# byteowlz/kokorox

Measured on NVIDIA B200. Metric: audio-seconds per second, higher is better.
Workload: dtype bf16

## Files before the change

### kokorox_b200/csrc/kernels.h

```cpp
#pragma once
#include "common.h"
#include <cuda_bf16.h>

namespace kkx {

enum Act : int { ACT_NONE = 0, ACT_LRELU = 1, ACT_SNAKE = 2, ACT_GELU_NEW = 3 };

struct ConvArgs {
  const float* in = nullptr; int ldi = 0;
  const int* in_off = nullptr; const int* in_len = nullptr;
  const int* m_len = nullptr; int max_m = 0; int B = 1;
  long long sum_m = 0;
  const float* w = nullptr; const float* bias = nullptr;
  int Ci = 0, Co = 0, ks = 1, dil = 1, pad = 0, stride = 1;
  const float* pscale = nullptr; const float* pshift = nullptr; int pld = 0;
  int pact = ACT_NONE; float pslope = 0.f; const float* palpha = nullptr;
  float* out = nullptr; int ldo = 0; int ocol = 0; const int* out_off = nullptr;
  int ors = 1, oro = 0;
  int eact = ACT_NONE;
  const float* res = nullptr; int ldr = 0; int rcol = 0; const int* res_off = nullptr;
  int res_shift = 0;
  float oscale = 1.f; int accumulate = 0;
};
void launch_conv_f32(const ConvArgs& a, cudaStream_t st);

struct TcConvArgs {
  const void* tmA = nullptr;
  const void* tmB = nullptr;
  const void* tmA2 = nullptr;
  const void* tmB2 = nullptr;
  const void* tmB_c = nullptr;
  const void* tmB2_c = nullptr;
  int debug = 0;
  int tf32 = 0;
  int nprod = 3;
  int f16 = 0;
  float wscale = 1.f;
  int eact = ACT_NONE;
  int Cpad = 0, Ci = 0, Co = 0, ks = 1, dil = 1, pad = 0;
  const int* in_off = nullptr; const int* m_len = nullptr; int max_m = 0; int B = 1; long long sum_m = 0;
  const float* bias = nullptr;
  float* out = nullptr; int ldo = 0; int ocol = 0; const int* out_off = nullptr; int ors = 1, oro = 0;
  const float* res = nullptr; int ldr = 0; int rcol = 0; const int* res_off = nullptr; int res_shift = 0;
  float oscale = 1.f; int accumulate = 0; int vec4 = 0;
  long long* timing = nullptr;
  const int* tile_start = nullptr; int ntiles_m = 0;
  int group_m = 1;
  void* out_hi = nullptr; void* out_lo = nullptr; int out_pl_ld = 0;
  void* attn_pl[6] = {nullptr, nullptr, nullptr, nullptr, nullptr, nullptr};
  int pair = 0;
  int force_kernel = 0;
  int nphase = 1;
  int phase_pad[10] = {0};
  int phase_oro[10] = {0};
  int phase_loop = 0;
};
void launch_conv_tc(const TcConvArgs& a, cudaStream_t st);
bool conv_tc_takes_pair(const TcConvArgs& a);
void make_tmap_bf16(void* out_map, const void* ptr, long long inner, long long outer,
                    long long pitch_elems, int box_outer);
void make_tmap_f32(void* out_map, const void* ptr, long long inner, long long outer,
                   long long pitch_elems, int box_outer);
void make_tmap_f16(void* out_map, const void* ptr, long long inner, long long outer,
                   long long pitch_elems, int box_outer);
inline int tc_box_n(int Co) { return Co > 128 ? 256 : (Co > 64 ? 128 : 64); }
inline int tc_box_n_tf32(int Co) { return Co > 64 ? 128 : 64; }
void launch_apply_tf32(const float* x, int ldx, int C, const float* scale, const float* shift, int act,
                       float slope, float* out_hi, float* out_lo, int Cpad, int rows_total,
                       const int* off, const int* len, int B, int max_len, cudaStream_t st);
constexpr float kSplitF16Scale = 16.f;
float split_f16_host(const float* w, size_t n, unsigned short* hi, unsigned short* lo);
void launch_apply_f16x2(const float* x, int ldx, int C, const float* scale, const float* shift, int act,
                        float slope, void* out_hi, void* out_lo, int Cpad, int rows_total,
                        const int* off, const int* len, int B, int max_len, cudaStream_t st);
void launch_apply_bf16(const float* x, int ldx, int C, const float* scale, const float* shift, int act,
                       float slope, const float* alpha, void* out, int Cpad, int rows_total,
                       const int* off, const int* len, int B, int max_len, cudaStream_t st);
void launch_im2col_bf16(const float* in, int ldi, int C, int ks, int stride, int pad, void* out, int Cpad,
                        int rows_total, const int* in_off, const int* in_len, const int* out_off,
                        const int* out_len, int B, int max_out_len, cudaStream_t st, int force_generic = 0);
void launch_pool_up_bf16(const float* in, int ldi, const float* scale, const float* shift, float slope,
                         const float* w, const float* bias, int C, void* out, int Cpad, int rows_total,
                         const int* in_off, const int* in_len, const int* out_off, int B, int max_len,
                         cudaStream_t st);

struct ArbConvArgs {
  const void* x = nullptr; int in_bf16 = 0;
  const float* scale = nullptr; const float* shift = nullptr;
  const float* alpha = nullptr;
  const void* tmB = nullptr;
  int C = 0, ks = 1, dil = 1, pad = 0;
  const int* off = nullptr; const int* len = nullptr;
  const int* tile_start = nullptr;
  int B = 1; int total_tiles = 0; long long sum_m = 0;
  const float* bias = nullptr;
  __nv_bfloat16* out_bf16 = nullptr;
  float* out_f32 = nullptr;
  const float* res = nullptr; float oscale = 1.f; int accumulate = 0;
  int res_bf16 = 0;
  float* part = nullptr; int nchunk = 0;
  long long* timing = nullptr;
  int debug = 0;
  int post = 0, cout = 0, ldo = 0; float slope = 0.f;
};
int arb_tile_rows(int C);
bool arb_conv_supported(int C, int ks, int dil, int B);
void launch_arb_conv(const ArbConvArgs& a, cudaStream_t st);

struct LnArgs {
  const float* x = nullptr; int ldx = 0;
  const float* res = nullptr; int ldr = 0;
  const float* w = nullptr; const float* b = nullptr;
  const float* ada = nullptr; int ada_ld = 0; int ada_off = 0;
  float eps = 1e-5f; float slope = 1.f;
  float* out = nullptr; int ldo = 0; int ocol = 0;
  const int* off = nullptr; const int* len = nullptr; int B = 1; int max_len = 0; int C = 0;
  void* pl_hi = nullptr; void* pl_lo = nullptr; int pl_ld = 0;
};
void launch_layernorm(const LnArgs& a, cudaStream_t st);

void launch_albert_embed(const int* ids, const float* word, const float* pos, const float* type,
                         const float* lnw, const float* lnb, float* out, const int* off,
                         const int* len, int B, int max_len, cudaStream_t st);
void launch_embed_rows(const int* ids, const float* table, int C, float* out, int ldo,
                       const int* off, const int* len, int B, int max_len, cudaStream_t st);
void launch_bcast_cols(const float* vec, int ldv, int voff, int C, float* out, int ldo, int ocol,
                       const int* off, const int* len, int B, int max_len, cudaStream_t st);
void launch_copy_cols(const float* src, int lds, int scol, float* dst, int ldd, int dcol, int C,
                      const int* off, const int* len, int B, int max_len, cudaStream_t st);
void launch_add_rows(const float* a, const float* b, float* out, int C, const int* off,
                     const int* len, int B, int max_len, cudaStream_t st);
void launch_copy_row(float* u, int C, int dst_row, int src_row, const int* off, int B,
                     cudaStream_t st);

void launch_attention(const float* qkv, float* ctx, const int* off, const int* len, int B,
                      int max_len, cudaStream_t st);

size_t attention_umma_scratch_floats(int rows_total, int B);
void attention_timing_dump();
void launch_attention_umma(const float* qkv, float* scratch, float* ctx, const int* off, const int* len, int B,
                           int max_len, int rows_total, cudaStream_t st, bool planes_ready = false);
void attention_umma_planes(float* scratch, int rows_total, int B, void* (&pl)[6]);

void launch_lstm(const float* xproj, const float* whhT, float* out, int ldo, int ocol,
                 const int* off, const int* len, int B, cudaStream_t st, int variant = 1);

constexpr int kStatRows = 128;
// ... 75 lines not shown
```

### kokorox_b200/csrc/kernels_arb.cu

```cuda
#include "kernels.h"
#include "tc_ptx.cuh"
#include <type_traits>
#include <cstdlib>

namespace kkx {

namespace {

#ifdef KKX_ARB_TIMING
#define TIM_DECL(n) long long tim_acc[n] = {0}; long long tim_last = clock64(); const bool tim_on = a.timing && blockIdx.x == 0
#define TICK(slot) do { if (tim_on) { const long long now_ = clock64(); tim_acc[slot] += now_ - tim_last; tim_last = now_; } } while (0)
#define TIM_FLUSH(base, n) do { if (tim_on) for (int i_ = 0; i_ < (n); i_++) atomicAdd(reinterpret_cast<unsigned long long*>(a.timing) + (base) + i_, (unsigned long long)tim_acc[i_]); } while (0)
#else
#define TIM_DECL(n)
#define TICK(slot)
#define TIM_FLUSH(base, n)
#endif

#ifdef KKX_EXPERIMENTS
#define ARB_DBG(a, bit) ((a).debug & (bit))
#else
#define ARB_DBG(a, bit) (0)
#endif

constexpr int kArbThreads = 512;
constexpr int kArbMaxB = 512;

template <int BN>
struct ArbCfg {
  static constexpr bool T = BN == 128;
  static constexpr int MSUB = T ? 2 : 1;
  static constexpr int KCH = BN / 64;
  static constexpr int RA = MSUB * 128 + 56;
  static constexpr uint32_t A_SLOT = RA * 128;
  static constexpr int NA = 3;
  static constexpr uint32_t B_STAGE = BN * 128;
  static constexpr int NB = T ? 6 : 3;
  static constexpr int PITCH = 36;
  static constexpr uint32_t STG = T ? 0 : 2 * 128 * PITCH * 4;
  static constexpr uint32_t STAT = 4 * BN * 2 * 4;
  static constexpr uint32_t COEF = 3 * BN * 4;
  static constexpr int NBAR = 2 * NA + 2 * NB + 4;
  static constexpr uint32_t SMEM = NA * A_SLOT + NB * B_STAGE + STG + STAT + COEF + NBAR * 8 + 16 + (3 * kArbMaxB + 2) * 4 + 1024;
  static_assert(A_SLOT % 1024 == 0, "A slot must keep the 1024-byte swizzle alignment");
};

__device__ __forceinline__ uint32_t pack_bf16(float lo, float hi) {
  __nv_bfloat162 p = __floats2bfloat162_rn(lo, hi);
  return *reinterpret_cast<uint32_t*>(&p);
}

struct TileCur {
  int b, mt;
  __device__ __forceinline__ void init(const int* ts, int B, int tile) {
    int lo = 0, hi = B;
    while (hi - lo > 1) {
      const int mid = (lo + hi) >> 1;
      if (ts[mid] <= tile) lo = mid; else hi = mid;
    }
    b = lo; mt = tile - ts[lo];
  }
  __device__ __forceinline__ void next(const int* ts) {
    mt++;
    while (ts[b] + mt >= ts[b + 1]) { b++; mt = 0; if (ts[b] < 0) break; }
  }
};

template <int BN, bool CONV2, bool POST = false, int SB = 0, bool PB = false>
__global__ void __launch_bounds__(kArbThreads, 1) arb_conv_kernel(const __grid_constant__ CUtensorMap tmB, ArbConvArgs a) {
  using Cfg = ArbCfg<BN>;
  constexpr bool T = Cfg::T;
  constexpr int MSUB = Cfg::MSUB;
  static_assert(SB == 0 || (!POST && (CONV2 || SB == 1)), "stream-bf16 variants: conv1 SB=1, conv2 SB=1 (bf16 out) / SB=2 (fp32 out)");
  static_assert(!PB || (T && !CONV2 && !POST && SB == 0), "balanced-producer variant: conv1, transposed accumulator, fp32 input");
  constexpr bool XIN_BF = CONV2 || SB != 0;
  constexpr bool OUT_BF = !CONV2 || SB == 1;
  static_assert(!POST || (T && !CONV2), "post variant: transposed accumulator, fp32 input");
  constexpr int NEW = PB ? 4 : 8;
  constexpr int NPW = PB ? 8 : 14 - NEW;
  constexpr int kProdThreads = NPW * 32;
  constexpr int kProdRows = kProdThreads / 8;
  constexpr int KCH = Cfg::KCH, NA = Cfg::NA, NB = Cfg::NB, PITCH = Cfg::PITCH;
  constexpr int MT = MSUB * 128;
  extern __shared__ uint8_t smem_raw[];
  const uint32_t base = (smem_u32(smem_raw) + 1023u) & ~1023u;
  uint8_t* const gbase = smem_raw + (base - smem_u32(smem_raw));
  const uint32_t a_base = base;
  const uint32_t b_base = a_base + NA * Cfg::A_SLOT;
  const uint32_t stg_base = b_base + NB * Cfg::B_STAGE;
  const uint32_t stat_base = stg_base + Cfg::STG;
  const uint32_t coef_base = stat_base + Cfg::STAT;
  const uint32_t bar_base = coef_base + Cfg::COEF;
  const uint32_t tmem_slot = bar_base + Cfg::NBAR * 8;
  const uint32_t ts_base = tmem_slot + 16;
  auto fullA = [&](int s) { return bar_base + s * 8; };
  auto emptyA = [&](int s) { return bar_base + (NA + s) * 8; };
  auto fullB = [&](int s) { return bar_base + (2 * NA + s) * 8; };
  auto emptyB = [&](int s) { return bar_base + (2 * NA + NB + s) * 8; };
  auto tfull = [&](int j) { return bar_base + (2 * NA + 2 * NB + j) * 8; };
  auto tempty = [&](int j) { return bar_base + (2 * NA + 2 * NB + 2 + j) * 8; };
  int* const s_ts = reinterpret_cast<int*>(gbase + (ts_base - base));
  int* const s_len = s_ts + (kArbMaxB + 2);
  int* const s_off = s_len + kArbMaxB;

  const int warp = threadIdx.x >> 5, lane = threadIdx.x & 31;
  const int B = a.B;
#pragma unroll 1
  for (int i = threadIdx.x; i <= B + 1; i += kArbThreads) s_ts[i] = i <= B ? a.tile_start[i] : -1;
#pragma unroll 1
  for (int i = threadIdx.x; i < B; i += kArbThreads) { s_len[i] = a.len[i]; s_off[i] = a.off[i]; }

  if (warp == 0 && lane == 0) {
    asm volatile("prefetch.tensormap [%0];" ::"l"(&tmB) : "memory");
    for (int s = 0; s < NA; s++) { mbar_init(fullA(s), kProdThreads / 32); mbar_init(emptyA(s), 1); }
    for (int s = 0; s < NB; s++) { mbar_init(fullB(s), 1); mbar_init(emptyB(s), 1); }
    for (int j = 0; j < 2; j++) { mbar_init(tfull(j), 1); mbar_init(tempty(j), NEW); }
    asm volatile("fence.mbarrier_init.release.cluster;" ::: "memory");
    asm volatile("fence.proxy.async.shared::cta;" ::: "memory");
  }
  if (warp == 1) {
    asm volatile("tcgen05.alloc.cta_group::1.sync.aligned.shared::cta.b32 [%0], %1;" ::"r"(tmem_slot), "r"(512u) : "memory");
    asm volatile("tcgen05.relinquish_alloc_permit.cta_group::1.sync.aligned;" ::: "memory");
  }
  tc_fence_before();
  __syncthreads();
  tc_fence_after();
  uint32_t tmem_base;
  asm volatile("ld.shared.b32 %0, [%1];" : "=r"(tmem_base) : "r"(tmem_slot) : "memory");

  const int t_begin = (int)(((long long)a.total_tiles * blockIdx.x) / gridDim.x);
  const int t_end = (int)(((long long)a.total_tiles * (blockIdx.x + 1)) / gridDim.x);
  const int ks = a.ks, dil = a.dil, pad = a.pad;

  if (warp == 0) {
    if (lane == 0 && t_begin < t_end) {
      int g = 0;
      TIM_DECL(2);
      const bool resident = KCH * ks <= NB;
#pragma unroll 1
      for (int tile = t_begin; tile < (resident ? t_begin + 1 : t_end); tile++) {
#pragma unroll 1
        for (int c = 0; c < KCH; c++)
#pragma unroll 1
          for (int tap = 0; tap < ks; tap++, g++) {
            const int s = g % NB;
            mbar_wait(emptyB(s), (((uint32_t)(g / NB)) & 1u) ^ 1u);
            TICK(0);
            mbar_expect_tx(fullB(s), Cfg::B_STAGE);
            tma_load_2d(b_base + s * Cfg::B_STAGE, &tmB, tap * BN + c * 64, 0, fullB(s));
            TICK(1);
          }
      }
      TIM_FLUSH(0, 2);
    }
  } else if (warp == 1) {
    if (lane == 0 && t_begin < t_end) {
      constexpr uint32_t idesc = umma_idesc_bf16(128, BN);
      int gA = 0, gB = 0, ti = 0;
      TileCur cur;
      cur.init(s_ts, B, t_begin);
      const bool resident = KCH * ks <= NB;
      TIM_DECL(4);
#pragma unroll 1
      for (int tile = t_begin; tile < t_end; tile++, ti++) {
        const int rem = s_len[cur.b] - cur.mt * MT;
        (void)rem;
        const int buf = ti & 1;
        mbar_wait(tempty(buf), (((uint32_t)(ti >> 1)) & 1u) ^ 1u);
        tc_fence_after();
        TICK(0);
#pragma unroll 1
        for (int c = 0; c < KCH; c++, gA++) {
          const int sa = gA % NA;
          mbar_wait(fullA(sa), ((uint32_t)(gA / NA)) & 1u);
          tc_fence_after();
          TICK(1);
          const uint32_t slot = a_base + sa * Cfg::A_SLOT;
#pragma unroll 1
          for (int tap = 0; tap < ks; tap++, gB++) {
            const int sb = resident ? c * ks + tap : gB % NB;
            if (!resident || ti == 0) {
              mbar_wait(fullB(sb), resident ? 0u : ((uint32_t)(gB / NB)) & 1u);
              tc_fence_after();
            }
            TICK(2);
            const uint64_t bd = umma_desc_sw128(b_base + sb * Cfg::B_STAGE);
            if (T) {
              constexpr uint32_t idescT = umma_idesc_bf16(128, 256);
              const uint64_t xd = umma_desc_sw128(slot + (uint32_t)(tap * dil) * 128u);
              const uint32_t td = tmem_base + (uint32_t)(buf * 256);
#pragma unroll
              for (int k = 0; k < 4; k++)
                if (!ARB_DBG(a, 8)) umma_bf16(td, bd + (uint64_t)(2 * k), xd + (uint64_t)(2 * k), idescT, (c | tap | k) ? 1u : 0u);
            } else {
#pragma unroll
              for (int sub = 0; sub < MSUB; sub++) {
                if (sub * 128 >= rem) continue;
                const uint64_t ad = umma_desc_sw128(slot + (uint32_t)(sub * 128 + tap * dil) * 128u);
                const uint32_t td = tmem_base + (uint32_t)((buf * MSUB + sub) * BN);
#pragma unroll
                for (int k = 0; k < 4; k++)
                  umma_bf16(td, ad + (uint64_t)(2 * k), bd + (uint64_t)(2 * k), idesc, (c | tap | k) ? 1u : 0u);
              }
            }
            if (!resident) umma_commit(emptyB(sb));
            TICK(3);
          }
          umma_commit(emptyA(sa));
        }
        umma_commit(tfull(buf));
        cur.next(s_ts);
      }
      TIM_FLUSH(4, 4);
    }
  } else if (T && warp < 2 + NEW) {
    const int eg = (warp - 2) >> 2;
    const int q = warp & 3;
    const int co = q * 32 + lane;
    const float bias_c = a.bias[co];
    const float2 bias2 = make_float2(bias_c, bias_c);
    const float2 os2 = make_float2(a.oscale, a.oscale);
    const bool accum = a.accumulate != 0;
    constexpr int RW = MSUB * 128 / (NEW / 4);
    constexpr int NCHK = RW / 32;
    auto fetchT = [&](int L, int off, int m0, int ch, float (&rv)[32]) {
      if (!CONV2 || ARB_DBG(a, 2)) return;
      const int row = m0 + eg * RW + ch * 32;
      const int left = L - row;
      if (SB) {
        const __nv_bfloat16* rp = reinterpret_cast<const __nv_bfloat16*>(a.res) + (size_t)(off + row) * 128 + co;
#pragma unroll
        for (int j = 0; j < 32; j++)
          if (j < left) rv[j] = __bfloat162float(rp[j * 128]);
      } else {
        const float* rp = a.res + (size_t)(off + row) * 128 + co;
#pragma unroll
        for (int j = 0; j < 32; j++)
          if (j < left) {
            if (ARB_DBG(a, 32)) asm volatile("ld.global.L1::no_allocate.f32 %0, [%1];" : "=f"(rv[j]) : "l"(rp + j * 128));
            else rv[j] = rp[j * 128];
          }
      }
    };
    int ti = 0;
    TileCur cur;
    float rv0[32], rv1[32];
    if (t_begin < t_end) {
      cur.init(s_ts, B, t_begin);
      fetchT(s_len[cur.b], s_off[cur.b], cur.mt * MT, 0, rv0);
      fetchT(s_len[cur.b], s_off[cur.b], cur.mt * MT, 1, rv1);
    }
#ifdef KKX_ARB_TIMING
    long long tim_acc[9] = {0}; long long tim_last = clock64();
    const bool tim_on = a.timing && blockIdx.x == 0 && warp == 2 && lane == 0;
#endif
#pragma unroll 1
    for (int tile = t_begin; tile < t_end; tile++, ti++) {
      const int b = cur.b;
      const int L = s_len[b], off = s_off[b];
      const int m0 = cur.mt * MT;
      const int buf = ti & 1;
      cur.next(s_ts);
      const bool has_next = tile + 1 < t_end;
      const int nL = has_next ? s_len[cur.b] : 0, noff = has_next ? s_off[cur.b] : 0, nm0 = cur.mt * MT;
      TICK(8);
      mbar_wait(tfull(buf), ((uint32_t)(ti >> 1)) & 1u);
      tc_fence_after();
// ... 333 lines not shown
        uint32_t pw[4];
#pragma unroll
        for (int e = 0; e < 4; e++) {
          if (POST) {
            const float2 lx = __fmul2_rn(xv[e], make_float2(a.slope, a.slope));
            pw[e] = pack_bf16(fmaxf(xv[e].x, lx.x), fmaxf(xv[e].y, lx.y)) & inmask;
            continue;
          }
          if (ARB_DBG(a, 4)) { pw[e] = pack_bf16(xv[e].x, xv[e].y) & inmask; continue; }
          const float2 u = __ffma2_rn(xv[e], cA[e], cB[e]);
          const float2 sn = make_float2(__sinf(u.x), __sinf(u.y));
          const float2 y = __fmul2_rn(__ffma2_rn(sn, sn, u), cI[e]);
          pw[e] = pack_bf16(y.x, y.y) & inmask;
        }
        const uint4 pk = make_uint4(pw[0], pw[1], pw[2], pw[3]);
        if (rloc + p * kProdRows < ra_used) *reinterpret_cast<uint4*>(sp + p * kProdRows * 128) = pk;
      }
      TICK(3);
      if (++s_g == ngc) {
        asm volatile("fence.proxy.async.shared::cta;" ::: "memory");
        __syncwarp();
        if (lane == 0) asm volatile("mbarrier.arrive.shared::cta.b64 _, [%0];" ::"r"(fullA(sa)) : "memory");
        s_g = 0; gA++;
        if (++s_c == KCH) { s_c = 0; sc_.next(s_ts); }
      }
    };

    Raw bufA[GP][RPP], bufB[GP][RPP];
#pragma unroll
    for (int p = 0; p < GP; p++)
#pragma unroll
      for (int v = 0; v < RPP; v++) { bufA[p][v] = Raw(); bufB[p][v] = Raw(); }
    if (F > 0) issue(bufA);
#pragma unroll 1
    for (int f = 0; f < F; f += 2) {
      if (f + 1 < F) issue(bufB);
      TICK(0);
      process(bufA);
      if (f + 1 >= F) break;
      if (f + 2 < F) issue(bufA);
      TICK(0);
      process(bufB);
    }
    TIM_FLUSH(20, 5);
  }
  tc_fence_before();
  __syncthreads();
  if (warp == 1) {
    tc_fence_after();
    asm volatile("tcgen05.dealloc.cta_group::1.sync.aligned.b32 %0, %1;" ::"r"(tmem_base), "r"(512u) : "memory");
  }
}

template <int BN, bool CONV2, bool POST = false, int SB = 0, bool PB = false>
void launch_arb_t(const ArbConvArgs& a, cudaStream_t st) {
  using Cfg = ArbCfg<BN>;
  static DevOnce once;
  int dev = 0;
  cudaGetDevice(&dev);
  once.run(dev, [] { KKX_CUDA(cudaFuncSetAttribute(arb_conv_kernel<BN, CONV2, POST, SB, PB>, cudaFuncAttributeMaxDynamicSharedMemorySize, (int)Cfg::SMEM)); });
  const int nsm = device_sm_count(dev);
  const int grid = a.total_tiles < nsm ? a.total_tiles : nsm;
  arb_conv_kernel<BN, CONV2, POST, SB, PB><<<grid, kArbThreads, Cfg::SMEM, st>>>(*reinterpret_cast<const CUtensorMap*>(a.tmB), a);
}

}

int arb_tile_rows(int C) { return (C == 128 ? ArbCfg<128>::MSUB : ArbCfg<256>::MSUB) * 128; }

bool arb_conv_supported(int C, int ks, int dil, int B) {
  return (C == 128 || C == 256) && ks >= 1 && dil >= 1 && dil * (ks - 1) <= 50 && (ks & 1) && B <= kArbMaxB;
}

void launch_arb_conv(const ArbConvArgs& a, cudaStream_t st) {
  if (g_dry_run) return;
  if (a.total_tiles <= 0 || a.B <= 0) return;
  if (!arb_conv_supported(a.C, a.ks, a.dil, a.B)) throw ArgError("launch_arb_conv: unsupported shape");
  if (a.post) {
    if (a.C != 128 || a.in_bf16 || !a.out_f32 || a.out_bf16 || a.res || a.accumulate || a.part || a.cout < 1 || a.cout > 128 ||
        a.ldo < a.cout || !(a.slope > 0.f && a.slope < 1.f))
      throw ArgError("launch_arb_conv: unsupported post-conv arguments");
    if (g_launch_stats) g_launch_stats->conv_flops += 2.0 * (double)a.sum_m * a.C * a.cout * a.ks;
    launch_arb_t<128, false, true>(a, st);
    post_launch("post_conv", st);
    return;
  }
  const bool conv2 = a.res != nullptr;
  if (conv2 ? (!a.in_bf16 || (a.out_f32 != nullptr) == (a.out_bf16 != nullptr) || (a.out_bf16 && (!a.res_bf16 || a.accumulate)))
            : (!a.out_bf16 || a.out_f32 || a.accumulate || a.res_bf16))
    throw ArgError("launch_arb_conv: unsupported input/output combination");
#ifdef KKX_EXPERIMENTS
  static const int dbg = env_int("KKX_ARB_DBG", 0);
  if (dbg && !a.debug) { ArbConvArgs d = a; d.debug = dbg; launch_arb_conv(d, st); return; }
#endif
  const bool stream_bf = conv2 ? a.res_bf16 != 0 : a.in_bf16 != 0;
  if (g_launch_stats) {
    const double fl = 2.0 * (double)a.sum_m * a.C * a.C * a.ks;
    g_launch_stats->conv_flops += fl;
    g_launch_stats->arb_flops += fl;
    const double bytes = conv2 ? 2.0 + (a.res_bf16 ? 2.0 : 4.0) + (a.out_bf16 ? 2.0 : 4.0) : (a.in_bf16 ? 2.0 : 4.0) + 2.0;
    g_launch_stats->arb_bytes += (double)a.sum_m * a.C * bytes;
  }
  if (stream_bf) {
    if (a.C == 128) {
      if (!conv2) launch_arb_t<128, false, false, 1>(a, st);
      else if (a.out_bf16) launch_arb_t<128, true, false, 1>(a, st);
      else launch_arb_t<128, true, false, 2>(a, st);
    } else {
      if (!conv2) launch_arb_t<256, false, false, 1>(a, st);
      else if (a.out_bf16) launch_arb_t<256, true, false, 1>(a, st);
      else launch_arb_t<256, true, false, 2>(a, st);
    }
  } else if (a.C == 128) {
    if (a.in_bf16) launch_arb_t<128, true>(a, st); else launch_arb_t<128, false, false, 0, true>(a, st);
  } else {
    if (a.in_bf16) launch_arb_t<256, true>(a, st); else launch_arb_t<256, false>(a, st);
  }
  if (g_launch_stats && g_launch_stats->profile && g_launch_stats->detail) {
    char nm[96]; snprintf(nm, sizeof nm, "arb_conv[c%d k%d d%d %s%s m%lld]", a.C, a.ks, a.dil, conv2 ? "conv2" : "conv1", stream_bf ? " sb" : "", a.sum_m);
    post_launch(nm, st);
  } else post_launch("arb_conv", st);
}

}
```

### kokorox_b200/csrc/kernels_tc.cu

```cuda
#include "kernels.h"
#include <cuda.h>
#include <cuda_bf16.h>
#include <cuda_fp16.h>
#include <mutex>
#include "tc_ptx.cuh"

#ifdef KKX_TC_DEBUG
#define TC_DBG(a, bit) ((a).debug & (bit))
#else
#define TC_DBG(a, bit) (0)
#endif

namespace kkx {

#ifdef KKX_TC_TIMING
#define TCT_DECL(n) long long tct_acc[n] = {0}; long long tct_last = clock64(); const bool tct_on = a.timing && blockIdx.x == gridDim.x - 2 && blockIdx.y == gridDim.y - 1 && blockIdx.z == gridDim.z - 1
#define TCT(slot) do { if (tct_on) { const long long now_ = clock64(); tct_acc[slot] += now_ - tct_last; tct_last = now_; } } while (0)
#define TCT_FLUSH(base, n) do { if (tct_on) for (int i_ = 0; i_ < (n); i_++) atomicAdd(reinterpret_cast<unsigned long long*>(a.timing) + (base) + i_, (unsigned long long)tct_acc[i_]); } while (0)
#else
#define TCT_DECL(n)
#define TCT(slot)
#define TCT_FLUSH(base, n)
#endif

typedef CUresult (*EncodeTiledFn)(CUtensorMap*, CUtensorMapDataType, cuuint32_t, void*, const cuuint64_t*,
                                  const cuuint64_t*, const cuuint32_t*, const cuuint32_t*,
                                  CUtensorMapInterleave, CUtensorMapSwizzle, CUtensorMapL2promotion,
                                  CUtensorMapFloatOOBfill);
static EncodeTiledFn get_encode() {
  static EncodeTiledFn fn = nullptr;
  static std::once_flag once;
  std::call_once(once, [] {
    void* p = nullptr;
    cudaDriverEntryPointQueryResult q;
    if (cudaGetDriverEntryPoint("cuTensorMapEncodeTiled", &p, cudaEnableDefault, &q) == cudaSuccess &&
        q == cudaDriverEntryPointSuccess)
      fn = (EncodeTiledFn)p;
  });
  if (!fn) throw CudaError("cuTensorMapEncodeTiled entry point not available");
  return fn;
}

static void make_tmap(void* out_map, const void* ptr, long long inner, long long outer,
                      long long pitch_elems, int box_outer, bool f32, bool f16 = false) {
  const int esz = f32 ? 4 : 2;
  cuuint64_t dims[2] = {(cuuint64_t)inner, (cuuint64_t)outer};
  cuuint64_t strides[1] = {(cuuint64_t)pitch_elems * esz};
  cuuint32_t box[2] = {(cuuint32_t)(128 / esz), (cuuint32_t)box_outer};
  cuuint32_t estr[2] = {1, 1};
  CUresult r = get_encode()((CUtensorMap*)out_map, f32 ? CU_TENSOR_MAP_DATA_TYPE_FLOAT32 : (f16 ? CU_TENSOR_MAP_DATA_TYPE_FLOAT16 : CU_TENSOR_MAP_DATA_TYPE_BFLOAT16), 2, const_cast<void*>(ptr),
                            dims, strides, box, estr, CU_TENSOR_MAP_INTERLEAVE_NONE, CU_TENSOR_MAP_SWIZZLE_128B,
                            CU_TENSOR_MAP_L2_PROMOTION_L2_256B, CU_TENSOR_MAP_FLOAT_OOB_FILL_NONE);
  if (r != CUDA_SUCCESS) {
    char b[160];
    snprintf(b, sizeof b, "cuTensorMapEncodeTiled failed (%d) inner=%lld outer=%lld pitch=%lld", (int)r, inner, outer, pitch_elems);
    throw CudaError(b);
  }
}
void make_tmap_bf16(void* out_map, const void* ptr, long long inner, long long outer,
                    long long pitch_elems, int box_outer) {
  make_tmap(out_map, ptr, inner, outer, pitch_elems, box_outer, false);
}
void make_tmap_f32(void* out_map, const void* ptr, long long inner, long long outer,
                   long long pitch_elems, int box_outer) {
  make_tmap(out_map, ptr, inner, outer, pitch_elems, box_outer, true);
}

void make_tmap_f16(void* out_map, const void* ptr, long long inner, long long outer,
                   long long pitch_elems, int box_outer) {
  make_tmap(out_map, ptr, inner, outer, pitch_elems, box_outer, false, true);
}

__device__ __forceinline__ float gelu_new_f(float v) {
  const float u = 0.7978845608028654f * (v + 0.044715f * v * v * v);
  return 0.5f * v * (1.0f + tanhf(u));
}

template <int BN, int STAGES, int MODE>
__global__ void __launch_bounds__(192) conv_tc_kernel(const __grid_constant__ CUtensorMap tmA,
                                                      const __grid_constant__ CUtensorMap tmB,
                                                      const __grid_constant__ CUtensorMap tmA2,
                                                      const __grid_constant__ CUtensorMap tmB2,
                                                      TcConvArgs a) {
  constexpr uint32_t PLANES = MODE ? 2 : 1;
  const int KE = (MODE && !a.f16) ? 32 : 64;
  const bool f16 = MODE && a.f16;
  const int cs = f16 ? 0 : 1;
  constexpr uint32_t A_BYTES = 128 * 128, B_BYTES = BN * 128, STAGE_BYTES = PLANES * (A_BYTES + B_BYTES);
  extern __shared__ uint8_t smem_raw[];
  const uint32_t base = (smem_u32(smem_raw) + 1023u) & ~1023u;
  constexpr uint32_t TMEM_COLS = MODE ? 4 * BN : BN;
  const uint32_t bar_base = base + STAGES * STAGE_BYTES;
  const uint32_t tmem_slot = bar_base + (2 * STAGES + 1 + 6) * 8;
  auto full_bar = [&](int s) { return bar_base + s * 8; };
  auto empty_bar = [&](int s) { return bar_base + (STAGES + s) * 8; };
  const uint32_t tfull_bar = bar_base + 2 * STAGES * 8;
  auto bfull_bar = [&](int j) { return bar_base + (2 * STAGES + 1 + j) * 8; };
  auto bempty_bar = [&](int j) { return bar_base + (2 * STAGES + 4 + j) * 8; };

  const int b = blockIdx.z;
  const int mlen = a.m_len[b];
  const bool fused = MODE == 0 && a.nphase > 1;
  const int bx = fused ? blockIdx.y : blockIdx.x, by = fused ? blockIdx.x : blockIdx.y;
  const int m0 = bx * 128;
  if (m0 >= mlen) return;
  const int ntn = (a.Co + BN - 1) / BN;
  const int ph = fused ? by / ntn : 0;
  const int c_pad = fused ? a.phase_pad[ph] : a.pad;
  const int c_oro = fused ? a.phase_oro[ph] : a.oro;
  const int n0 = (fused ? by - ph * ntn : by) * BN;
  const int wrow0 = ph * a.Co + n0;
  const int warp = threadIdx.x >> 5, lane = threadIdx.x & 31;
  const int kchunks = a.Cpad / KE;
  const int num_k = a.ks * kchunks;

  if (warp == 0 && lane == 0) {
    asm volatile("prefetch.tensormap [%0];" ::"l"(&tmA) : "memory");
    asm volatile("prefetch.tensormap [%0];" ::"l"(&tmB) : "memory");
    if (MODE) {
      asm volatile("prefetch.tensormap [%0];" ::"l"(&tmA2) : "memory");
      asm volatile("prefetch.tensormap [%0];" ::"l"(&tmB2) : "memory");
    }
    for (int s = 0; s < STAGES; s++) { mbar_init(full_bar(s), 1); mbar_init(empty_bar(s), 1); }
// ... 1865 lines not shown
```

### kokorox_b200/csrc/model_forward.cu

```cuda
#include "model.h"
#include <algorithm>
#include <cmath>
#include <cstdlib>

namespace kkx {

namespace {
long long* g_arb_timing = nullptr;
long long* arb_timing_buf() {
  static const bool on = env_flag("KKX_ARB_TIMING", false);
  if (!on) return nullptr;
  if (!g_arb_timing) {
    KKX_CUDA(cudaMalloc(&g_arb_timing, 128 * sizeof(long long)));
    KKX_CUDA(cudaMemset(g_arb_timing, 0, 128 * sizeof(long long)));
  }
  return g_arb_timing;
}
ConvArgs gemm_args(const Level& L, const float* in, int ldi, int K, const float* w, const float* bias,
                   int N, float* out, int ldo, int ocol) {
  ConvArgs a;
  a.in = in; a.ldi = ldi; a.in_off = L.d_off; a.in_len = L.d_len;
  a.m_len = L.d_len; a.max_m = L.max_len; a.B = L.B; a.sum_m = L.sum_len;
  a.w = w; a.bias = bias; a.Ci = K; a.Co = N;
  a.out = out; a.ldo = ldo; a.ocol = ocol; a.out_off = L.d_off;
// ... 376 lines not shown
    if (w.w1x1) {
      void* a3 = A.alloc_bytes((size_t)Lin.rows * cpi * 2);
      float* s = A.alloc<float>((size_t)Lin.rows * w.co);
      launch_apply_bf16(x, ldx, w.ci, nullptr, nullptr, ACT_NONE, 0.f, nullptr, a3, cpi, Lin.rows, Lin.d_off,
                        Lin.d_len, B, Lin.max_len, st);
      tc_conv(A, a3, Lin.rows, w.t1x1, 1, 0, Lin, Lin, nullptr, s, w.co, 0, Lin, 1, 0, nullptr, 0, nullptr, 0, 1.f, false);
      scp = s; ldsc = w.co;
    }
    tc_conv(A, a2, Lout.rows, w.t2, 1, 1, Lout, Lout, w.b2, out, ldo, ocol, Lout, 1, 0, scp, ldsc, &Lin,
            w.up ? 1 : 0, 0.70710678118654752440f, false);
    return;
  }
  if (w.up) {
    float* p = A.alloc<float>((size_t)Lout.rows * w.ci);
    launch_pool_up(x, ldx, sc1, sh1, 0.2f, w.poolw, w.poolb, w.ci, p, w.ci, Lin.d_off, Lin.d_len,
                   Lout.d_off, B, Lin.max_len, st);
    gemm(Lout, Lout, p, w.ci, w.ci, w.w1, &w.s1, w.b1, w.co, t, w.co, 0, ACT_NONE, 3, 1);
  } else {
    gemm(Lin, Lin, x, ldx, w.ci, w.w1, &w.s1, w.b1, w.co, t, w.co, 0, ACT_NONE, 3, 1, sc1, sh1, ACT_LRELU, 0.2f);
  }
  launch_colstats(t, w.co, w.co, part, Lout.d_off, Lout.d_len, B, Lout.max_len, st);
  launch_adain_coef(part, w.co, Lout.max_len, Lout.d_len, sty, sld, w.sty2, 1e-5f, sc2, sh2, B, st);

  const float* sc = x; int ldsc = ldx;
  if (w.w1x1) {
    float* s = A.alloc<float>((size_t)Lin.rows * w.co);
    gemm(Lin, Lin, x, ldx, w.ci, w.w1x1, &w.s1x1, nullptr, w.co, s, w.co, 0);
    sc = s; ldsc = w.co;
  }
  gemm(Lout, Lout, t, w.co, w.co, w.w2, &w.s2, w.b2, w.co, out, ldo, ocol, ACT_NONE, 3, 1, sc2, sh2, ACT_LRELU, 0.2f,
       sc, ldsc, &Lin, w.up ? 1 : 0, 0.70710678118654752440f);
}

bool Model::use_stream_bf16(int C, int k, int B) const {
  return opt.precision == 1 && opt.stream_bf16 && arb_conv_supported(C, k, 5, B);
}

void Model::arb(Run& r, Arena& A, const ArbW& w, const float* x, const Level& L, const float* sty,
                int sld, float* xw, float* t1, float* out, float oscale, bool accumulate, const float* part_x,
                const void* x_bf16) {
  (void)r;
  cudaStream_t st = cur_;
  const int B = L.B, C = w.c, k = w.k;
  const int nch = (L.max_len + kStatRows - 1) / kStatRows;
  float* part = A.alloc<float>((size_t)B * nch * 2 * C);
  float* sc = A.alloc<float>((size_t)B * C);
  float* sh = A.alloc<float>((size_t)B * C);
  const int dil[3] = {1, 3, 5};
  const float* cur = x;
  const bool tc = opt.precision == 1;
  void* abuf = tc ? A.alloc_bytes((size_t)L.rows * w.t1[0].Cpad * 2) : nullptr;
  if (tc) {
    ArbConvArgs base;
    base.C = C; base.ks = k; base.off = L.d_off; base.len = L.d_len; base.B = B; base.sum_m = L.sum_len;
    const bool t256 = arb_tile_rows(C) == 256;
    base.tile_start = t256 ? L.d_tiles256 : L.d_tiles128;
    base.total_tiles = t256 ? L.ntiles256 : L.ntiles128;
    base.scale = sc; base.shift = sh; base.nchunk = nch;
    const bool sb = use_stream_bf16(C, k, B);
    void* xb0 = nullptr;
    if (sb && !x_bf16) xb0 = A.alloc_bytes((size_t)L.rows * C * 2);
    if (!part_x) launch_colstats(cur, C, C, part, L.d_off, L.d_len, B, L.max_len, st, xb0);
    else if (sb && !x_bf16) throw ArgError("arb: a bf16 stream with caller-provided statistics needs the bf16 input too");
    const void* curb = sb ? (x_bf16 ? x_bf16 : xb0) : nullptr;
    long long* tim = arb_timing_buf();
    static const int tim_ks = env_int("KKX_ARB_TIMING_KS", 0);
    if (tim_ks && tim_ks != k) tim = nullptr;
    for (int j = 0; j < 3; j++) {
      launch_adain_coef(j == 0 && part_x ? part_x : part, C, L.max_len, L.d_len, sty, sld, w.s1[j], 1e-5f, sc, sh, B, st);
      ArbConvArgs c1 = base;
      if (tim) c1.timing = tim + (C == 128 ? 0 : 64);
      c1.x = sb ? curb : (const void*)cur; c1.in_bf16 = sb ? 1 : 0; c1.alpha = w.a1[j]; c1.tmB = w.t1[j].tmap; c1.dil = dil[j];
      c1.pad = dil[j] * (k - 1) / 2; c1.bias = w.b1[j];
      c1.out_bf16 = static_cast<__nv_bfloat16*>(abuf); c1.part = part;
      launch_arb_conv(c1, st);
      launch_adain_coef(part, C, L.max_len, L.d_len, sty, sld, w.s2[j], 1e-5f, sc, sh, B, st);
      float* dst = (j == 2) ? out : xw;
      ArbConvArgs c2 = base;
      if (tim) c2.timing = tim + (C == 128 ? 32 : 96);
      c2.x = abuf; c2.in_bf16 = 1; c2.alpha = w.a2[j]; c2.tmB = w.t2[j].tmap; c2.dil = 1; c2.pad = (k - 1) / 2;
      c2.bias = w.b2[j];
      if (sb) {
        c2.res = static_cast<const float*>(curb); c2.res_bf16 = 1;
        if (j == 2) { c2.out_f32 = out; c2.oscale = oscale; c2.accumulate = accumulate ? 1 : 0; }
        else { c2.out_bf16 = reinterpret_cast<__nv_bfloat16*>(xw); c2.part = part; curb = xw; }
      } else {
        c2.out_f32 = dst; c2.res = cur;
        if (j == 2) { c2.oscale = oscale; c2.accumulate = accumulate ? 1 : 0; } else c2.part = part;
      }
      launch_arb_conv(c2, st);
      cur = dst;
    }
    return;
  }
  for (int j = 0; j < 3; j++) {
    launch_colstats(cur, C, C, part, L.d_off, L.d_len, B, L.max_len, st);
    launch_adain_coef(part, C, L.max_len, L.d_len, sty, sld, w.s1[j], 1e-5f, sc, sh, B, st);
    ConvArgs c1 = gemm_args(L, cur, C, C, w.w1[j], w.b1[j], C, t1, C, 0);
    c1.ks = k; c1.dil = dil[j]; c1.pad = dil[j] * (k - 1) / 2;
    c1.pscale = sc; c1.pshift = sh; c1.pld = C; c1.pact = ACT_SNAKE; c1.palpha = w.a1[j];
    launch_conv_f32(c1, st);
    launch_colstats(t1, C, C, part, L.d_off, L.d_len, B, L.max_len, st);
    launch_adain_coef(part, C, L.max_len, L.d_len, sty, sld, w.s2[j], 1e-5f, sc, sh, B, st);
    float* dst = (j == 2) ? out : xw;
    ConvArgs c2 = gemm_args(L, t1, C, C, w.w2[j], w.b2[j], C, dst, C, 0);
    c2.ks = k; c2.dil = 1; c2.pad = (k - 1) / 2;
    c2.pscale = sc; c2.pshift = sh; c2.pld = C; c2.pact = ACT_SNAKE; c2.palpha = w.a2[j];
// ... 366 lines not shown
```

### kokorox_b200/csrc/testapi.cu

```cuda
#include "../../include/kkx_test.h"
#include "kernels.h"
#include "model.h"
#include <algorithm>
#include <cstring>
#include <limits>
#include <string>
#include <vector>

using namespace kkx;
static thread_local std::string t_err;

namespace {
struct DevBuf {
  void* p = nullptr;
  DevBuf(const void* host, size_t bytes) {
    KKX_CUDA(cudaMalloc(&p, bytes ? bytes : 4));
    if (host && bytes) KKX_CUDA(cudaMemcpy(p, host, bytes, cudaMemcpyHostToDevice));
  }
  ~DevBuf() { if (p) cudaFree(p); }
  template <class T> T* as() { return static_cast<T*>(p); }
};
template <class F> int run(int device, F&& f) {
  try {
    int n = 0;
// ... 473 lines not shown
static inline uint16_t host_bf16(float f) {
  uint32_t u; memcpy(&u, &f, 4);
  return (uint16_t)((u + 0x7FFFu + ((u >> 16) & 1u)) >> 16);
}

}

static int arb_conv_test(int device, const float* x, int B, const int* lens, int C, int in_bf16,
                         const float* scale, const float* shift, const float* alpha, const float* w,
                         const float* bias, int ks, int dil, const float* res, int res_bf16, float oscale,
                         int accumulate, int want_bf16, float* out, float* sums, int desc_mode) {
  return run(device, [&] {
    if (!arb_conv_supported(C, ks, dil, B)) throw ArgError("kkx_test_arb_conv: unsupported shape");
    std::vector<int> off(B), tiles(B + 1, 0);
    const int MT = arb_tile_rows(C);
    int o = kGapRows, maxL = 0; long long sumL = 0;
    for (int b = 0; b < B; b++) {
      off[b] = o; o = (o + lens[b] + kGapRows + 7) & ~7;
      tiles[b + 1] = tiles[b] + (lens[b] + MT - 1) / MT;
      maxL = std::max(maxL, lens[b]); sumL += lens[b];
    }
    const int rows = o;
    const float qnan = std::numeric_limits<float>::quiet_NaN();
    std::vector<float> hx((size_t)rows * C, qnan), hres((size_t)rows * C, qnan), hout((size_t)rows * C, qnan);
    size_t src = 0;
    for (int b = 0; b < B; b++) {
      memcpy(hx.data() + (size_t)off[b] * C, x + src * C, (size_t)lens[b] * C * 4);
      if (res) memcpy(hres.data() + (size_t)off[b] * C, res + src * C, (size_t)lens[b] * C * 4);
      memcpy(hout.data() + (size_t)off[b] * C, out + src * C, (size_t)lens[b] * C * 4);
      src += lens[b];
    }
    std::vector<uint16_t> hxb;
    if (in_bf16) { hxb.resize(hx.size()); for (size_t i = 0; i < hx.size(); i++) hxb[i] = host_bf16(hx[i]); }
    std::vector<uint16_t> hw((size_t)C * ks * C);
    for (size_t i = 0; i < hw.size(); i++) hw[i] = host_bf16(w[i]);
    DevBuf dx(in_bf16 ? (const void*)hxb.data() : (const void*)hx.data(), hx.size() * (in_bf16 ? 2 : 4));
    DevBuf dw(hw.data(), hw.size() * 2), db(bias, C * 4), dsc(scale, (size_t)B * C * 4), dsh(shift, (size_t)B * C * 4);
    std::vector<uint16_t> hresb;
    if (res && res_bf16) { hresb.resize(hres.size()); for (size_t i = 0; i < hres.size(); i++) hresb[i] = host_bf16(hres[i]); }
    DevBuf dal(alpha, C * 4), dres(res ? (res_bf16 ? (const void*)hresb.data() : (const void*)hres.data()) : nullptr,
                                   res ? hres.size() * (res_bf16 ? 2 : 4) : 0);
    DevBuf dout(hout.data(), hout.size() * 4), doutb(nullptr, hout.size() * 2);
    KKX_CUDA(cudaMemset(doutb.p, 0xFF, hout.size() * 2));
    const int nchunk = (maxL + 127) / 128;
    DevBuf dpart(nullptr, (size_t)B * nchunk * 2 * C * 4);
    KKX_CUDA(cudaMemset(dpart.p, 0, (size_t)B * nchunk * 2 * C * 4));
    DevBuf doff(off.data(), B * 4), dlen(lens, B * 4), dts(tiles.data(), (B + 1) * 4);
    alignas(64) unsigned char tmB[128];
    make_tmap_bf16(tmB, dw.p, (long long)ks * C, C, (long long)ks * C, tc_box_n(C));
    ArbConvArgs a;
    a.x = dx.p; a.in_bf16 = in_bf16; a.scale = dsc.as<float>(); a.shift = dsh.as<float>(); a.alpha = dal.as<float>();
    a.tmB = tmB; a.C = C; a.ks = ks; a.dil = dil; a.pad = dil * (ks - 1) / 2;
    a.off = doff.as<int>(); a.len = dlen.as<int>(); a.tile_start = dts.as<int>(); a.B = B; a.total_tiles = tiles[B];
    a.sum_m = sumL; a.bias = db.as<float>();
    a.out_bf16 = want_bf16 ? doutb.as<__nv_bfloat16>() : nullptr;
    a.out_f32 = want_bf16 ? nullptr : dout.as<float>();
    a.res = res ? dres.as<float>() : nullptr; a.res_bf16 = res ? res_bf16 : 0; a.oscale = oscale; a.accumulate = accumulate;
    a.part = sums ? dpart.as<float>() : nullptr; a.nchunk = nchunk; (void)desc_mode;
    launch_arb_conv(a, 0);
    KKX_CUDA(cudaDeviceSynchronize());
    if (want_bf16) {
      std::vector<uint16_t> hb(hout.size());
      KKX_CUDA(cudaMemcpy(hb.data(), doutb.p, hb.size() * 2, cudaMemcpyDeviceToHost));
      for (size_t i = 0; i < hb.size(); i++) { uint32_t u = (uint32_t)hb[i] << 16; memcpy(&hout[i], &u, 4); }
    } else {
      KKX_CUDA(cudaMemcpy(hout.data(), dout.p, hout.size() * 4, cudaMemcpyDeviceToHost));
    }
    src = 0;
    for (int b = 0; b < B; b++) {
      memcpy(out + src * C, hout.data() + (size_t)off[b] * C, (size_t)lens[b] * C * 4);
      src += lens[b];
    }
    if (sums) {
      std::vector<float> hp((size_t)B * nchunk * 2 * C);
      KKX_CUDA(cudaMemcpy(hp.data(), dpart.p, hp.size() * 4, cudaMemcpyDeviceToHost));
      for (int b = 0; b < B; b++)
        for (int k = 0; k < 2; k++)
          for (int c = 0; c < C; c++) {
            double acc = 0.0;
            for (int ch = 0; ch < (lens[b] + 127) / 128; ch++) acc += hp[(((size_t)b * nchunk + ch) * 2 + k) * C + c];
            sums[((size_t)b * 2 + k) * C + c] = (float)acc;
          }
    }
  });
}

extern "C" {

KKX_API int kkx_test_arb_conv(int device, const float* x, int B, const int* lens, int C, int in_bf16,
                              const float* scale, const float* shift, const float* alpha, const float* w,
                              const float* bias, int ks, int dil, const float* res, float oscale,
                              int accumulate, int want_bf16, float* out, float* sums, int desc_mode) {
  return arb_conv_test(device, x, B, lens, C, in_bf16, scale, shift, alpha, w, bias, ks, dil, res, 0, oscale, accumulate,
                       want_bf16, out, sums, desc_mode);
}

KKX_API int kkx_test_arb_conv_stream(int device, const float* x, int B, const int* lens, int C, const float* scale,
                                     const float* shift, const float* alpha, const float* w, const float* bias, int ks,
                                     int dil, const float* res, float oscale, int accumulate, int want_bf16, float* out,
                                     float* sums) {
  return arb_conv_test(device, x, B, lens, C, 1, scale, shift, alpha, w, bias, ks, dil, res, 1, oscale, accumulate,
                       want_bf16, out, sums, 0);
}

}
```

Measured before the change: 10700.

## Add TMA-based residual load and store epilogue for C=128 conv2

Result: no change. 10700 (median of 6 runs) (-0.0%).

```diff
diff --git a/kokorox_b200/csrc/kernels.h b/kokorox_b200/csrc/kernels.h
--- a/kokorox_b200/csrc/kernels.h
+++ b/kokorox_b200/csrc/kernels.h
@@ -63,6 +63,7 @@
                    long long pitch_elems, int box_outer);
 void make_tmap_f16(void* out_map, const void* ptr, long long inner, long long outer,
                    long long pitch_elems, int box_outer);
+void make_tmap_f32_rows(void* out_map, const void* ptr, long long inner, long long outer, int box_outer);
 inline int tc_box_n(int Co) { return Co > 128 ? 256 : (Co > 64 ? 128 : 64); }
 inline int tc_box_n_tf32(int Co) { return Co > 64 ? 128 : 64; }
 void launch_apply_tf32(const float* x, int ldx, int C, const float* scale, const float* shift, int act,
@@ -93,6 +94,7 @@
   const int* off = nullptr; const int* len = nullptr;
   const int* tile_start = nullptr;
   int B = 1; int total_tiles = 0; long long sum_m = 0;
+  int rows = 0;
   const float* bias = nullptr;
   __nv_bfloat16* out_bf16 = nullptr;
   float* out_f32 = nullptr;
diff --git a/kokorox_b200/csrc/kernels_arb.cu b/kokorox_b200/csrc/kernels_arb.cu
--- a/kokorox_b200/csrc/kernels_arb.cu
+++ b/kokorox_b200/csrc/kernels_arb.cu
@@ -26,23 +26,30 @@
 constexpr int kArbThreads = 512;
 constexpr int kArbMaxB = 512;
 
-template <int BN>
+template <int BN, bool TE = false>
 struct ArbCfg {
   static constexpr bool T = BN == 128;
+  static_assert(!TE || T, "TMA epilogue: transposed accumulator only");
   static constexpr int MSUB = T ? 2 : 1;
   static constexpr int KCH = BN / 64;
-  static constexpr int RA = MSUB * 128 + 56;
+  static constexpr int HALO = TE ? 16 : 56;
+  static constexpr int RA = MSUB * 128 + HALO;
   static constexpr uint32_t A_SLOT = RA * 128;
-  static constexpr int NA = 3;
+  static constexpr int NA = TE ? 2 : 3;
   static constexpr uint32_t B_STAGE = BN * 128;
   static constexpr int NB = T ? 6 : 3;
   static constexpr int PITCH = 36;
   static constexpr uint32_t STG = T ? 0 : 2 * 128 * PITCH * 4;
-  static constexpr uint32_t STAT = 4 * BN * 2 * 4;
+  static constexpr uint32_t STAT = TE ? 0 : 4 * BN * 2 * 4;
   static constexpr uint32_t COEF = 3 * BN * 4;
-  static constexpr int NBAR = 2 * NA + 2 * NB + 4;
-  static constexpr uint32_t SMEM = NA * A_SLOT + NB * B_STAGE + STG + STAT + COEF + NBAR * 8 + 16 + (3 * kArbMaxB + 2) * 4 + 1024;
+  static constexpr int RB = 16;
+  static constexpr uint32_t RBOX = RB * BN * 4;
+  static constexpr int NRT = TE ? 6 : 0;
+  static constexpr uint32_t RING = NRT * RBOX;
+  static constexpr int NBAR = 2 * NA + 2 * NB + 4 + NRT;
+  static constexpr uint32_t SMEM = NA * A_SLOT + NB * B_STAGE + RING + STG + STAT + COEF + NBAR * 8 + 16 + (3 * kArbMaxB + 2) * 4 + 1024;
   static_assert(A_SLOT % 1024 == 0, "A slot must keep the 1024-byte swizzle alignment");
+  static_assert(SMEM <= 232448, "shared memory per block");
 };
 
 __device__ __forceinline__ uint32_t pack_bf16(float lo, float hi) {
@@ -66,13 +73,15 @@
   }
 };
 
-template <int BN, bool CONV2, bool POST = false, int SB = 0, bool PB = false>
-__global__ void __launch_bounds__(kArbThreads, 1) arb_conv_kernel(const __grid_constant__ CUtensorMap tmB, ArbConvArgs a) {
-  using Cfg = ArbCfg<BN>;
+template <int BN, bool CONV2, bool POST = false, int SB = 0, bool PB = false, bool TE = false>
+__global__ void __launch_bounds__(kArbThreads, 1) arb_conv_kernel(const __grid_constant__ CUtensorMap tmB, const __grid_constant__ CUtensorMap tmR,
+                                                                  const __grid_constant__ CUtensorMap tmO, ArbConvArgs a) {
+  using Cfg = ArbCfg<BN, TE>;
   constexpr bool T = Cfg::T;
   constexpr int MSUB = Cfg::MSUB;
+  static_assert(!TE || (CONV2 && !POST && SB == 0), "TMA epilogue: conv2 with an fp32 residual stream");
   static_assert(SB == 0 || (!POST && (CONV2 || SB == 1)), "stream-bf16 variants: conv1 SB=1, conv2 SB=1 (bf16 out) / SB=2 (fp32 out)");
-  static_assert(!PB || (T && !CONV2 && !POST && SB == 0), "balanced-producer variant: conv1, transposed accumulator, fp32 input");
+  static_assert(!PB || (T && !POST && SB == 0 && (!CONV2 || TE)), "balanced-producer variant: conv1 (fp32 input) or conv2 with the TMA epilogue");
   constexpr bool XIN_BF = CONV2 || SB != 0;
   constexpr bool OUT_BF = !CONV2 || SB == 1;
   static_assert(!POST || (T && !CONV2), "post variant: transposed accumulator, fp32 input");
@@ -87,7 +96,8 @@
   uint8_t* const gbase = smem_raw + (base - smem_u32(smem_raw));
   const uint32_t a_base = base;
   const uint32_t b_base = a_base + NA * Cfg::A_SLOT;
-  const uint32_t stg_base = b_base + NB * Cfg::B_STAGE;
+  const uint32_t ring_base = b_base + NB * Cfg::B_STAGE;
+  const uint32_t stg_base = ring_base + Cfg::RING;
   const uint32_t stat_base = stg_base + Cfg::STG;
   const uint32_t coef_base = stat_base + Cfg::STAT;
   const uint32_t bar_base = coef_base + Cfg::COEF;
@@ -99,6 +109,8 @@
   auto emptyB = [&](int s) { return bar_base + (2 * NA + NB + s) * 8; };
   auto tfull = [&](int j) { return bar_base + (2 * NA + 2 * NB + j) * 8; };
   auto tempty = [&](int j) { return bar_base + (2 * NA + 2 * NB + 2 + j) * 8; };
+  constexpr int NR = TE ? Cfg::NRT / (NEW / 4) : 0;
+  auto rfull = [&](int g, int s) { return bar_base + (2 * NA + 2 * NB + 4 + g * NR + s) * 8; };
   int* const s_ts = reinterpret_cast<int*>(gbase + (ts_base - base));
   int* const s_len = s_ts + (kArbMaxB + 2);
   int* const s_off = s_len + kArbMaxB;
@@ -115,6 +127,12 @@
     for (int s = 0; s < NA; s++) { mbar_init(fullA(s), kProdThreads / 32); mbar_init(emptyA(s), 1); }
     for (int s = 0; s < NB; s++) { mbar_init(fullB(s), 1); mbar_init(emptyB(s), 1); }
     for (int j = 0; j < 2; j++) { mbar_init(tfull(j), 1); mbar_init(tempty(j), NEW); }
+    for (int g = 0; g < NEW / 4; g++)
+      for (int s = 0; s < NR; s++) mbar_init(rfull(g, s), 1);
+    if (TE) {
+      asm volatile("prefetch.tensormap [%0];" ::"l"(&tmR) : "memory");
+      asm volatile("prefetch.tensormap [%0];" ::"l"(&tmO) : "memory");
+    }
     asm volatile("fence.mbarrier_init.release.cluster;" ::: "memory");
     asm volatile("fence.proxy.async.shared::cta;" ::: "memory");
   }
@@ -213,6 +231,140 @@
       }
       TIM_FLUSH(4, 4);
     }
+  } else if (TE && warp < 2 + NEW) {
+    constexpr int RB = Cfg::RB;
+    constexpr int SLACK = NR >= 6 ? 2 : 1;
+    constexpr int LEAD = NR - SLACK;
+    constexpr int RW = MSUB * 128 / (NEW / 4);
+    constexpr int NCHK = RW / 32;
+    constexpr int NH = RW / RB;
+    const int eg = (warp - 2) >> 2;
+    const int q = warp & 3;
+    const int co = q * 32 + lane;
+    const bool leader = warp == 2 + 4 * eg && lane == 0;
+    const float bias_c = a.bias[co];
+    const float2 bias2 = make_float2(bias_c, bias_c);
+    const float2 os2 = make_float2(a.oscale, a.oscale);
+    const bool accum = a.accumulate != 0;
+    const uint32_t ring_s = ring_base + (uint32_t)(eg * NR) * Cfg::RBOX;
+    float* const ring = reinterpret_cast<float*>(gbase + (ring_s - base)) + co;
+    TileCur lc = {0, 0}; int lh = 0, ls = 0, nl = 0;
+    const int nbox = (t_end - t_begin) * NH;
+    auto load_next = [&]() {
+      const int row = lc.mt * MT + eg * RW + lh * RB;
+      if (row < s_len[lc.b]) {
+        mbar_expect_tx(rfull(eg, ls), Cfg::RBOX);
+        tma_load_2d(ring_s + (uint32_t)ls * Cfg::RBOX, &tmR, 0, s_off[lc.b] + row, rfull(eg, ls));
+      } else {
+        asm volatile("mbarrier.arrive.shared::cta.b64 _, [%0];" ::"r"(rfull(eg, ls)) : "memory");
+      }
+      nl++;
+      if (++ls == NR) ls = 0;
+      if (++lh == NH) { lh = 0; lc.next(s_ts); }
+    };
+    int ti = 0, cs = 0;
+    uint32_t cph = 0;
+    TileCur cur;
+    if (t_begin < t_end) {
+      cur.init(s_ts, B, t_begin);
+      if (leader) { lc = cur; while (nl < LEAD && nl < nbox) load_next(); }
+    }
+#ifdef KKX_ARB_TIMING
+    long long tim_acc[9] = {0}; long long tim_last = clock64();
+    const bool tim_on = a.timing && blockIdx.x == 0 && warp == 2 && lane == 0;
+#endif
+#pragma unroll 1
+    for (int tile = t_begin; tile < t_end; tile++, ti++) {
+      const int b = cur.b;
+      const int L = s_len[b], off = s_off[b];
+      const int m0 = cur.mt * MT;
+      const int buf = ti & 1;
+      cur.next(s_ts);
+      TICK(8);
+      mbar_wait(tfull(buf), ((uint32_t)(ti >> 1)) & 1u);
+      tc_fence_after();
+      TICK(0);
+      float2 s2 = make_float2(0.f, 0.f), q2 = s2;
+      auto bodyT = [&](int ch, auto full_tag) {
+        constexpr bool FULL = decltype(full_tag)::value;
+        const int row = m0 + eg * RW + ch * 32;
+        uint32_t v[32];
+        tmem_ld32(tmem_base + ((uint32_t)(q * 32) << 16) + (uint32_t)(buf * 256 + eg * RW + ch * 32), v);
+        if (ch == NCHK - 1) {
+          tc_fence_before();
+          if (lane == 0) asm volatile("mbarrier.arrive.shared::cta.b64 _, [%0];" ::"r"(tempty(buf)) : "memory");
+        }
+        TICK(1);
+#pragma unroll
+        for (int hh = 0; hh < 32 / RB; hh++) {
+          const int hrow = row + hh * RB;
+          const int left = L - hrow;
+          const bool whole = FULL || left >= RB;
+          mbar_wait(rfull(eg, cs), cph);
+          TICK(2);
+          float* const bx = ring + cs * (RB * BN);
+          float* const op = a.out_f32 + (size_t)(off + hrow) * 128 + co;
+#pragma unroll
+          for (int j = 0; j < RB; j += 2) {
+            float2 o = make_float2(__uint_as_float(v[hh * RB + j]), __uint_as_float(v[hh * RB + j + 1]));
+            o = __fadd2_rn(__fadd2_rn(o, make_float2(bx[j * BN], bx[(j + 1) * BN])), bias2);
+            if (!FULL) { o.x = j < left ? o.x : 0.f; o.y = j + 1 < left ? o.y : 0.f; }
+            s2 = __fadd2_rn(s2, o);
+            q2 = __ffma2_rn(o, o, q2);
+            o = __fmul2_rn(o, os2);
+            if (whole) {
+              bx[j * BN] = o.x; bx[(j + 1) * BN] = o.y;
+            } else if (accum) {
+              if (j < left) asm volatile("red.global.add.f32 [%0], %1;" ::"l"(op + j * 128), "f"(o.x) : "memory");
+              if (j + 1 < left) asm volatile("red.global.add.f32 [%0], %1;" ::"l"(op + (j + 1) * 128), "f"(o.y) : "memory");
+            } else {
+              if (j < left) op[j * 128] = o.x;
+              if (j + 1 < left) op[(j + 1) * 128] = o.y;
+            }
+          }
+          TICK(5);
+          asm volatile("fence.proxy.async.shared::cta;" ::: "memory");
+          asm volatile("bar.sync %0, 128;" ::"r"(1 + eg) : "memory");
+          TICK(4);
+          if (leader) {
+            if (whole) {
+              const uint32_t src = ring_s + (uint32_t)cs * Cfg::RBOX;
+              if (accum)
+                asm volatile("cp.reduce.async.bulk.tensor.2d.global.shared::cta.add.tile.bulk_group [%0, {%1, %2}], [%3];"
+                             ::"l"(&tmO), "r"(0), "r"(off + hrow), "r"(src) : "memory");
+              else
+                asm volatile("cp.async.bulk.tensor.2d.global.shared::cta.tile.bulk_group [%0, {%1, %2}], [%3];"
+                             ::"l"(&tmO), "r"(0), "r"(off + hrow), "r"(src) : "memory");
+            }
+            asm volatile("cp.async.bulk.commit_group;" ::: "memory");
+            if (nl < nbox) {
+              asm volatile("cp.async.bulk.wait_group.read %0;" ::"n"(SLACK) : "memory");
+              load_next();
+            }
+          }
+          TICK(6);
+          if (++cs == NR) { cs = 0; cph ^= 1u; }
+        }
+        if ((ch & 3) == 3) {
+          if (a.part && row - 96 < L) {
+            float* pp = a.part + ((size_t)b * a.nchunk + (size_t)((row - 96) >> 7)) * 2 * 128 + co;
+            pp[0] = s2.x + s2.y;
+            pp[128] = q2.x + q2.y;
+          }
+          s2 = make_float2(0.f, 0.f); q2 = s2;
+        }
+        TICK(7);
+      };
+      if (L - m0 >= MT) {
+#pragma unroll
+        for (int ch = 0; ch < NCHK; ch++) bodyT(ch, std::true_type{});
+      } else {
+#pragma unroll
+        for (int ch = 0; ch < NCHK; ch++) bodyT(ch, std::false_type{});
+      }
+    }
+    if (leader) asm volatile("cp.async.bulk.wait_group 0;" ::: "memory");
+    TIM_FLUSH(8, 9);
   } else if (T && warp < 2 + NEW) {
     const int eg = (warp - 2) >> 2;
     const int q = warp & 3;
@@ -652,16 +804,22 @@
   }
 }
 
-template <int BN, bool CONV2, bool POST = false, int SB = 0, bool PB = false>
+template <int BN, bool CONV2, bool POST = false, int SB = 0, bool PB = false, bool TE = false>
 void launch_arb_t(const ArbConvArgs& a, cudaStream_t st) {
-  using Cfg = ArbCfg<BN>;
+  using Cfg = ArbCfg<BN, TE>;
   static DevOnce once;
   int dev = 0;
   cudaGetDevice(&dev);
-  once.run(dev, [] { KKX_CUDA(cudaFuncSetAttribute(arb_conv_kernel<BN, CONV2, POST, SB, PB>, cudaFuncAttributeMaxDynamicSharedMemorySize, (int)Cfg::SMEM)); });
+  once.run(dev, [] { KKX_CUDA(cudaFuncSetAttribute(arb_conv_kernel<BN, CONV2, POST, SB, PB, TE>, cudaFuncAttributeMaxDynamicSharedMemorySize, (int)Cfg::SMEM)); });
+  alignas(64) unsigned char tmR[128] = {}, tmO[128] = {};
+  if (TE) {
+    make_tmap_f32_rows(tmR, a.res, BN, a.rows, Cfg::RB);
+    make_tmap_f32_rows(tmO, a.out_f32, BN, a.rows, Cfg::RB);
+  }
   const int nsm = device_sm_count(dev);
   const int grid = a.total_tiles < nsm ? a.total_tiles : nsm;
-  arb_conv_kernel<BN, CONV2, POST, SB, PB><<<grid, kArbThreads, Cfg::SMEM, st>>>(*reinterpret_cast<const CUtensorMap*>(a.tmB), a);
+  arb_conv_kernel<BN, CONV2, POST, SB, PB, TE><<<grid, kArbThreads, Cfg::SMEM, st>>>(
+      *reinterpret_cast<const CUtensorMap*>(a.tmB), *reinterpret_cast<const CUtensorMap*>(tmR), *reinterpret_cast<const CUtensorMap*>(tmO), a);
 }
 
 }
@@ -712,7 +870,16 @@
       else launch_arb_t<256, true, false, 2>(a, st);
     }
   } else if (a.C == 128) {
-    if (a.in_bf16) launch_arb_t<128, true>(a, st); else launch_arb_t<128, false, false, 0, true>(a, st);
+    if (a.in_bf16) {
+      if (a.dil * (a.ks - 1) <= ArbCfg<128, true>::HALO) {
+        if (a.rows <= 0) throw ArgError("launch_arb_conv: conv2 needs the row count of its tensors");
+        launch_arb_t<128, true, false, 0, true, true>(a, st);
+      } else {
+        launch_arb_t<128, true>(a, st);
+      }
+    } else {
+      launch_arb_t<128, false, false, 0, true>(a, st);
+    }
   } else {
     if (a.in_bf16) launch_arb_t<256, true>(a, st); else launch_arb_t<256, false>(a, st);
   }
diff --git a/kokorox_b200/csrc/kernels_tc.cu b/kokorox_b200/csrc/kernels_tc.cu
--- a/kokorox_b200/csrc/kernels_tc.cu
+++ b/kokorox_b200/csrc/kernels_tc.cu
@@ -69,6 +69,21 @@
 void make_tmap_f16(void* out_map, const void* ptr, long long inner, long long outer,
                    long long pitch_elems, int box_outer) {
   make_tmap(out_map, ptr, inner, outer, pitch_elems, box_outer, false, true);
+}
+
+void make_tmap_f32_rows(void* out_map, const void* ptr, long long inner, long long outer, int box_outer) {
+  cuuint64_t dims[2] = {(cuuint64_t)inner, (cuuint64_t)outer};
+  cuuint64_t strides[1] = {(cuuint64_t)inner * 4};
+  cuuint32_t box[2] = {(cuuint32_t)inner, (cuuint32_t)box_outer};
+  cuuint32_t estr[2] = {1, 1};
+  CUresult r = get_encode()((CUtensorMap*)out_map, CU_TENSOR_MAP_DATA_TYPE_FLOAT32, 2, const_cast<void*>(ptr), dims, strides, box,
+                            estr, CU_TENSOR_MAP_INTERLEAVE_NONE, CU_TENSOR_MAP_SWIZZLE_NONE, CU_TENSOR_MAP_L2_PROMOTION_L2_256B,
+                            CU_TENSOR_MAP_FLOAT_OOB_FILL_NONE);
+  if (r != CUDA_SUCCESS) {
+    char b[160];
+    snprintf(b, sizeof b, "cuTensorMapEncodeTiled failed (%d) rows: inner=%lld outer=%lld box=%d", (int)r, inner, outer, box_outer);
+    throw CudaError(b);
+  }
 }
 
 __device__ __forceinline__ float gelu_new_f(float v) {
diff --git a/kokorox_b200/csrc/model_forward.cu b/kokorox_b200/csrc/model_forward.cu
--- a/kokorox_b200/csrc/model_forward.cu
+++ b/kokorox_b200/csrc/model_forward.cu
@@ -452,7 +452,7 @@
   void* abuf = tc ? A.alloc_bytes((size_t)L.rows * w.t1[0].Cpad * 2) : nullptr;
   if (tc) {
     ArbConvArgs base;
-    base.C = C; base.ks = k; base.off = L.d_off; base.len = L.d_len; base.B = B; base.sum_m = L.sum_len;
+    base.C = C; base.ks = k; base.off = L.d_off; base.len = L.d_len; base.B = B; base.sum_m = L.sum_len; base.rows = L.rows;
     const bool t256 = arb_tile_rows(C) == 256;
     base.tile_start = t256 ? L.d_tiles256 : L.d_tiles128;
     base.total_tiles = t256 ? L.ntiles256 : L.ntiles128;
diff --git a/kokorox_b200/csrc/testapi.cu b/kokorox_b200/csrc/testapi.cu
--- a/kokorox_b200/csrc/testapi.cu
+++ b/kokorox_b200/csrc/testapi.cu
@@ -549,7 +549,7 @@
     a.x = dx.p; a.in_bf16 = in_bf16; a.scale = dsc.as<float>(); a.shift = dsh.as<float>(); a.alpha = dal.as<float>();
     a.tmB = tmB; a.C = C; a.ks = ks; a.dil = dil; a.pad = dil * (ks - 1) / 2;
     a.off = doff.as<int>(); a.len = dlen.as<int>(); a.tile_start = dts.as<int>(); a.B = B; a.total_tiles = tiles[B];
-    a.sum_m = sumL; a.bias = db.as<float>();
+    a.sum_m = sumL; a.rows = rows; a.bias = db.as<float>();
     a.out_bf16 = want_bf16 ? doutb.as<__nv_bfloat16>() : nullptr;
     a.out_f32 = want_bf16 ? nullptr : dout.as<float>();
     a.res = res ? dres.as<float>() : nullptr; a.res_bf16 = res ? res_bf16 : 0; a.oscale = oscale; a.accumulate = accumulate;
```
